# learningmatter-mit/surface-sampling

Hardware: AMD Instinct MI355X
Metric: MC energy-evaluations/sec (SrTiO3(001) ~250-atom slabs, 3-model PaiNN ensemble E+F incl. neighbor list) (higher is better)
Workload: dtype f32 via fp16x2-split MFMA (3 products), fp32 accumulate; neighbor decisions f64; 1 GPU; SrTiO3(001) PaiNN x3, 256 batched independent chains per GPU (BASELINE configs[3]), 248-272 atoms/chain; chains_per_gpu=256, atoms_per_gpu=66503, edges_per_gpu=2747786, slots_per_gpu=2836316, models=3, streams_per_gpu=2, parallelism=one GPU, no collective

## Files before the change

### surface-sampling_amd/csrc/api_painn.hip

```cpp
#include <cmath>

#include "vssr_internal.h"

namespace vssr {

static void transpose(const float *src, int rows, int cols, float *dst) {
    for (int r = 0; r < rows; ++r)
        for (int c = 0; c < cols; ++c) dst[(size_t)c * rows + r] = src[(size_t)r * cols + c];
}

static int upload_weights(vssr_handle *h, const vssr_painn_config *cfg) {
    const int M = cfg->n_models, L = cfg->num_conv, R = cfg->n_rbf, H = cfg->readout_hidden, NE = cfg->n_embed;
    const size_t per_layer = (size_t)F * F + F + (size_t)F3 * F + F3 + (size_t)F3 * R + F3 + 2 * (size_t)F * F +
                             (size_t)F * 2 * F + F + (size_t)F3 * F + F3;
    const size_t blob_len = (size_t)NE * F + L * per_layer + (size_t)H * F + H + H + 1;
    if (cfg->weights_len != blob_len)
        return set_err(h, VSSR_E_BADARG, "weights_len %llu does not match the layout (%zu floats)",
                       (unsigned long long)cfg->weights_len, blob_len);
    const size_t t_per_layer = (size_t)F * F + (size_t)F * F3 + 2 * (size_t)F * F + (size_t)2 * F * F + (size_t)F * F3;
    const size_t img_len = blob_len + L * t_per_layer + (size_t)F * H;
    std::vector<float> img(img_len * M);
    std::vector<ModelW> table(M);
    if (h->weights.ensure(img.size() * sizeof(float)))
        return set_err(h, VSSR_E_NOMEM, "weights: out of device memory");
// ... 83 lines not shown
        for (int m = 0; m < M; ++m) {
            const float *hb = img.data() + (size_t)m * img_len;
            size_t o = (size_t)NE * F;
            for (int l = 0; l < L; ++l) {
                const float *Wd = hb + o + (size_t)F * F + F + (size_t)F3 * F + F3;
                build_wd16(Wd, Wd + (size_t)F3 * 20, w16.data() + ((size_t)m * L + l) * per_layer16);
                o += per_layer;
            }
        }
        if (h->wd16.ensure(w16.size() * sizeof(unsigned))) return set_err(h, VSSR_E_NOMEM, "split filter weights");
        VSSR_HIP(h, hipMemcpy(h->wd16.p, w16.data(), w16.size() * sizeof(unsigned), hipMemcpyHostToDevice));
        for (int m = 0; m < M; ++m)
            for (int l = 0; l < L; ++l)
                table[m].layer[l].wd16 = h->wd16.as<uint4>() + ((size_t)m * L + l) * per_layer16 / 4;
    }
    {
        const size_t per_model = (size_t)NE * 2 * 24 * F;
        std::vector<float> A(per_model * M), At(per_model * M);
        for (int m = 0; m < M; ++m) {
            const float *hb = img.data() + (size_t)m * img_len;
            size_t o = (size_t)NE * F;
            const float *W1 = hb + o; o += (size_t)F * F;
            const float *b1 = hb + o; o += F;
            const float *W2 = hb + o; o += (size_t)F3 * F;
            const float *b2 = hb + o; o += F3;
            const float *Wd = hb + o; o += (size_t)F3 * R;
            const float *bd = hb + o;
            l0_build_tables(hb, W1, b1, W2, b2, Wd, bd, NE, A.data() + per_model * m, At.data() + per_model * m);
        }
        const size_t pk = l0_packed_dwords(NE);
        std::vector<unsigned> A16(pk * M), At16(pk * M);
        for (int m = 0; m < M; ++m) l0_pack_tables(A.data() + per_model * m, NE, A16.data() + pk * m, At16.data() + pk * m);
        if (h->d_l0A.ensure(A16.size() * sizeof(unsigned)) || h->d_l0At.ensure(At16.size() * sizeof(unsigned)))
            return set_err(h, VSSR_E_NOMEM, "layer-0 tables");
        VSSR_HIP(h, hipMemcpy(h->d_l0A.p, A16.data(), A16.size() * sizeof(unsigned), hipMemcpyHostToDevice));
        VSSR_HIP(h, hipMemcpy(h->d_l0At.p, At16.data(), At16.size() * sizeof(unsigned), hipMemcpyHostToDevice));
    }
    if (h->model_table.ensure(sizeof(ModelW) * M)) return set_err(h, VSSR_E_NOMEM, "model table");
    VSSR_HIP(h, hipMemcpy(h->model_table.p, table.data(), sizeof(ModelW) * M, hipMemcpyHostToDevice));
    return VSSR_OK;
}

}

using namespace vssr;

extern "C" {

int vssr_create(const vssr_painn_config *cfg, vssr_handle **out) {
    if (!cfg || !out) return set_err(nullptr, VSSR_E_BADARG, "null argument");
    *out = nullptr;
    if (cfg->struct_size != sizeof(vssr_painn_config))
        return set_err(nullptr, VSSR_E_BADARG, "vssr_painn_config size mismatch (%u vs %zu)", cfg->struct_size,
                       sizeof(vssr_painn_config));
    if (cfg->feat_dim < 16 || cfg->feat_dim > 256 || cfg->feat_dim % 16 != 0 || cfg->n_rbf < 1 || cfg->n_rbf > 32)
        return set_err(nullptr, VSSR_E_BADARG,
                       "feat_dim must be a multiple of 16 in 16..256 and n_rbf in 1..32 (got %d, %d)", cfg->feat_dim, cfg->n_rbf);
    if (cfg->n_models < 1 || cfg->n_models > MAX_MODELS || cfg->num_conv < 1 || cfg->num_conv > MAX_LAYERS ||
        cfg->readout_hidden < 1 || cfg->readout_hidden > F || cfg->n_embed < 1 || !cfg->weights ||
        !(cfg->cutoff > 0) || !(cfg->model_units_per_ev > 0))
        return set_err(nullptr, VSSR_E_BADARG, "bad PaiNN configuration");
    if (cfg->excl_vol && (cfg->excl_power < 1 || cfg->excl_power > 64 || !(cfg->excl_sigma > 0)))
        return set_err(nullptr, VSSR_E_BADARG, "excluded volume: power %d (1 .. 64) / sigma %g out of range", cfg->excl_power,
                       (double)cfg->excl_sigma);
    return create_handle(Kind::PAINN, cfg->device, out, [cfg](vssr_handle *h) {
        h->n_models = cfg->n_models; h->n_rbf = cfg->n_rbf; h->num_conv = cfg->num_conv; h->n_embed = cfg->n_embed;
        h->readout_hidden = cfg->readout_hidden; h->cutoff = cfg->cutoff; h->excl_vol = cfg->excl_vol;
        h->excl_power = cfg->excl_power; h->excl_sigma = cfg->excl_sigma; h->units_per_ev = cfg->model_units_per_ev;
        h->feat_dim = cfg->feat_dim;
        h->painn_general = !(cfg->feat_dim == F && cfg->n_rbf == 20);
        if (const char *e = getenv("VSSR_PAINN_PATH")) h->painn_general = h->painn_general || strcmp(e, "general") == 0;
        int rc = VSSR_OK;
        if (h->painn_general) {
            h->l0_enabled = 0;
            rc = painn_gen_upload(h, cfg);
        } else {
            rc = upload_weights(h, cfg);
            if (!rc) rc = node_mfma_init(h);
            if (!rc) rc = edge_mfma_init(h);
            if (!rc) rc = l0_mfma_init(h);
        }
        if (const char *e = getenv("VSSR_EDGE_IMPL")) h->edge_impl = (strcmp(e, "gather") == 0) ? 0 : 1;
        if (const char *e = getenv("VSSR_L0_FACTORISE")) h->l0_enabled = h->painn_general ? 0 : atoi(e);
        if (const char *e = getenv("VSSR_UPD_SAVE")) h->upd_save = atoi(e);
        if (const char *e = getenv("VSSR_DEBUG_KEEP")) h->debug_keep = atoi(e);
        if (const char *e = getenv("VSSR_EDGE_FS16_MAX")) h->fs16_max_atoms = atoi(e);
        if (const char *e = getenv("VSSR_EDGE_FS8_MAX")) h->fs8_max_atoms = atoi(e);
        if (const char *e = getenv("VSSR_EDGE_BWD_MPASS")) h->bwd_multi_pass = atoi(e);
        if (const char *e = getenv("VSSR_EDGE_SUB_CHUNK")) { const int c = atoi(e); if (c >= 8) { h->sub_chunk_fwd = c; h->sub_chunk_bwd = c; } }
        if (const char *e = getenv("VSSR_EDGE_FWD_2PASS")) { const int w = atoi(e); h->fwd_two_pass = (w == 8 || w == 16) ? w : w ? 16 : 0; }
        if (!rc && cfg->offset_per_z) {
            h->has_offset = true;
            h->offset_const = cfg->offset_const;
            if (h->offset_per_z.ensure(sizeof(double) * cfg->n_embed)) rc = set_err(h, VSSR_E_NOMEM, "offset table");
            else if (hipMemcpy(h->offset_per_z.p, cfg->offset_per_z, sizeof(double) * cfg->n_embed,
                               hipMemcpyHostToDevice) != hipSuccess)
                rc = set_err(h, VSSR_E_DEVICE, "offset table upload failed");
        }
        return rc;
    });
}

}
```

### surface-sampling_amd/csrc/painn.hip

```cpp
#include "vssr_internal.h"

namespace vssr {

constexpr int T = NODE_TILE;
constexpr int RB = 21;
constexpr int ECHUNK = 16;
constexpr float PI_F = 3.14159265358979323846f;

__device__ inline float sigmoidf_(float x) { return 1.f / (1.f + expf(-x)); }
__device__ inline float swishf_(float x) { return x * sigmoidf_(x); }
__device__ inline float dswishf_(float x) {
    float sg = sigmoidf_(x);
    return sg * fmaf(x, 1.f - sg, 1.f);
}

__global__ void __launch_bounds__(128) k_embed(int N, const int *__restrict__ Z, const ModelW *__restrict__ MW,
                                               float *__restrict__ s0, float *__restrict__ v0) {
    int i = blockIdx.x, m = blockIdx.y, f = threadIdx.x;
    const ModelW &W = MW[m];
    size_t a = (size_t)m * N + i;
    s0[a * F + f] = W.embed[(size_t)Z[i] * F + f];
    v0[(a * 3 + 0) * F + f] = 0.f;
    v0[(a * 3 + 1) * F + f] = 0.f;
    v0[(a * 3 + 2) * F + f] = 0.f;
// ... 504 lines not shown
    sv.n_atoms = (int)N;
    sv.n_models = (int)M;
    for (size_t l = 0; l <= L; ++l) { sv.s_in[l] = p; p += nS; sv.v_in[l] = p; p += nV; }
    for (size_t l = 0; l < L; ++l) {
        sv.phi[l] = p; p += nP;
        sv.s_msg[l] = p; p += nS;
        sv.v_msg[l] = p; p += nV;
    }
    sv.e_atom = p; p += M * N;
    sv.sbar = p; p += nS;
    sv.vbar = p; p += nV;
    sv.sbar_msg = p; p += nS;
    sv.vbar_msg = p; p += nV;
    sv.phibar = p; p += nP;
    if (h->upd_save && readout_mfma_supported(h->readout_hidden) &&
        h->d_upd_save.ensure(update_save_bytes((int)N, (int)M) * L))
        return set_err(h, VSSR_E_NOMEM, "forward intermediates of the update blocks: out of device memory");
    const size_t groups = (size_t)painn_gbar_groups(h);
    const bool compact = h->gbar_mode == 2 && groups > 1;
    if (h->d_gbar.ensure(sizeof(float4) * M * (compact ? 1 : groups) * (size_t)h->slot_cap) ||
        (compact && h->d_gpart.ensure(sizeof(float) * 3 * M * groups * (size_t)h->slot_cap + 256)))
        return set_err(h, VSSR_E_NOMEM, "edge-gradient buffer: out of device memory");
    sv.gbar = h->d_gbar.as<float4>();
    return painn_alloc_results(h);
}

int painn_alloc_results(vssr_handle *h) {
    const size_t N = h->n_atoms, M = h->n_models;
    if (h->d_energy.ensure(sizeof(float) * h->n_cfg) || h->d_energy_std.ensure(sizeof(float) * h->n_cfg) ||
        h->d_energy_models.ensure(sizeof(float) * h->n_cfg * M) || h->d_energy64.ensure(sizeof(double) * h->n_cfg * (2 + M)) ||
        h->d_forces.ensure(sizeof(float) * 3 * N) ||
        h->d_forces_std.ensure(sizeof(float) * 3 * N) || h->d_e_atoms.ensure(sizeof(float) * N))
        return set_err(h, VSSR_E_NOMEM, "result buffers: out of device memory");
    if (h->d_sat.bytes < sizeof(unsigned) * h->n_cfg || h->d_sat_out.bytes < sizeof(unsigned) * h->n_cfg) {
        if (h->d_sat.ensure(sizeof(unsigned) * h->n_cfg) || h->d_sat_out.ensure(sizeof(unsigned) * h->n_cfg))
            return set_err(h, VSSR_E_NOMEM, "saturation flags: out of device memory");
        VSSR_HIP(h, hipMemsetAsync(h->d_sat.p, 0, h->d_sat.bytes, h->stream));
        VSSR_HIP(h, hipMemsetAsync(h->d_sat_out.p, 0, h->d_sat_out.bytes, h->stream));
    }
    return VSSR_OK;
}

int painn_run(vssr_handle *h, uint32_t want) {
    if (h->painn_general) return painn_gen_run(h, want);
    const int N = h->n_atoms, M = h->n_models, L = h->num_conv, H = h->readout_hidden;
    hipStream_t st = h->stream;
    h->h_sat_valid = false;
    int rc = build_neighbors(h, (double)h->cutoff);
    if (rc) return rc;
    rc = painn_alloc_state(h);
    if (rc) return rc;
    StateView &sv = h->sv;
    sv.e_excl = h->d_excl.as<float>();
    GraphView G;
    G.n_atoms = N;
    G.n_cfg = h->n_cfg;
    G.atom_cfg = h->d_atom_cfg.as<int>();
    G.cfg_start = h->d_cfg_start.as<int>();
    G.row_start = h->d_row_start.as<int>();
    G.deg = h->d_deg.as<int>();
    G.edge = h->d_edge.as<float4>();
    G.rev = h->d_rev.as<int>();
    G.erec = h->d_erec.as<float4>();
    G.rho = h->d_rho.as<float>();
    G.dist2 = h->d_dist.as<float2>();
    G.rho16 = h->d_rho16.as<uint4>();
    G.drho16 = h->d_drho16.as<uint4>();
    G.zslot = h->d_zslot.as<unsigned char>();
    G.bundle = h->d_bundle.as<int4>();
    G.chain_class = h->d_chain_class.as<unsigned char>();
    G.act = ActiveView{h->active_mask, h->d_atom_cfg.as<int>(), h->d_sat.as<unsigned>()};
    const ActiveView &av = G.act;
    const ModelW *MW = h->model_table.as<ModelW>();
    const int *counters = h->d_counters.as<int>();
    const int *Z = h->d_Z.as<int>();
    dim3 blk(128);
    dim3 g_atom(N, M), g_tile((N + T - 1) / T, M);
    Profiler &P = h->prof;
    const bool l0_fact = h->l0_enabled && h->l0_nz > 0;
    const int n_groups = painn_gbar_groups(h);
    const int layer_sets = n_groups > 1 ? gbar_layer_sets(h) : 1;
    const bool compact = h->gbar_mode == 2 && n_groups > 1;
    const int fin_groups = compact ? 1 : n_groups;
    const int *cls_list[EDGE_MFMA_CLASSES];
    const int *bcls_list[EDGE_MFMA_BCLASSES];
    {
        int o = 0;
        for (int c = 0; c < EDGE_MFMA_CLASSES; o += h->n_class[c], ++c) cls_list[c] = h->d_class_list.as<int>() + o;
        for (int c = 0; c < EDGE_MFMA_BCLASSES; o += h->n_bclass[c], ++c) bcls_list[c] = h->d_class_list.as<int>() + o;
    }
    const int n_gather = h->n_class[EDGE_CLASS_GATHER];
    const bool keep = h->upd_save && (want & VSSR_WANT_FORCES) && readout_mfma_supported(H);
    auto save_of = [&](int l) -> void * { return keep ? (char *)h->d_upd_save.p + update_save_bytes(N, M) * (size_t)l : nullptr; };
    h->l0_used = l0_fact;

    if (!l0_fact) {
        P.begin(KC_EMBED, st);
        hipLaunchKernelGGL(k_embed, g_atom, blk, 0, st, N, Z, MW, sv.s_in[0], sv.v_in[0]);
        P.end(st);
    }
    for (int l = 0; l < L; ++l) {
        if (l == 0 && l0_fact) {
            P.begin(KC_L0_FWD, st);
            rc = l0_run_forward(h, G, sv.s_msg[0], sv.v_msg[0]);
            if (rc) return rc;
            P.end(st);
            P.begin(KC_UPDATE_FWD, st);
            launch_update_fwd_mfma(st, N, M, l, av, MW, sv.s_msg[l], sv.v_msg[l], sv.s_in[l + 1],
                                   (l + 1 < L || h->debug_keep) ? sv.v_in[l + 1] : nullptr, l + 1 < L ? sv.phi[l + 1] : nullptr, save_of(l));
            P.end(st);
            continue;
        }
        if (l == 0) {
            P.begin(KC_MSG_MLP, st);
            launch_msg_mlp_mfma(st, N, M, l, av, MW, sv.s_in[l], sv.phi[l]);
            P.end(st);
        }
        P.begin(KC_EDGE_FWD, st);
        if (l == 0)
            hipLaunchKernelGGL(k_edge_fwd<true>, g_atom, blk, 0, st, N, l, MW, G, counters, h->cutoff, h->excl_vol,
                               h->excl_sigma, h->excl_power, sv.s_in[l], sv.v_in[l], sv.phi[l], sv.s_msg[l],
                               sv.v_msg[l], -1);
        else {
            for (int cls = 0; cls < EDGE_MFMA_CLASSES; ++cls)
                launch_edge_fwd_mfma(st, cls, N, cls_list[cls], h->n_class[cls], M, l, h->max_class_atoms[cls], MW, G, counters,
                                     (int)(h->slot_cap - 1), sv.s_in[l], sv.v_in[l], sv.phi[l], sv.s_msg[l], sv.v_msg[l],
                                     (cls == EDGE_CLASS_FS4 && h->fwd_two_pass) ? h->d_bundle_sub.as<int4>() : (const int4 *)nullptr,
                                     h->fwd_two_pass, h->sub_chunk_fwd ? h->sub_chunk_fwd : sub_chunk_max(h->fwd_two_pass));
            if (n_gather)
                hipLaunchKernelGGL(k_edge_fwd<false>, g_atom, blk, 0, st, N, l, MW, G, counters, h->cutoff, h->excl_vol,
                                   h->excl_sigma, h->excl_power, sv.s_in[l], sv.v_in[l], sv.phi[l], sv.s_msg[l],
                                   sv.v_msg[l], (int)EDGE_BCLASS_GATHER);
        }
        P.end(st);
        P.begin(KC_UPDATE_FWD, st);
        launch_update_fwd_mfma(st, N, M, l, av, MW, sv.s_msg[l], sv.v_msg[l], sv.s_in[l + 1],
                               (l + 1 < L || h->debug_keep) ? sv.v_in[l + 1] : nullptr, l + 1 < L ? sv.phi[l + 1] : nullptr, save_of(l));
        P.end(st);
    }
    const bool fused = readout_mfma_supported(H);
    const bool want_forces = (want & VSSR_WANT_FORCES) != 0;
    const float *e_excl = h->excl_vol ? sv.e_excl : (const float *)nullptr;
    if (!(fused && want_forces)) {
        P.begin(KC_READOUT, st);
        if (fused) launch_readout_mfma(st, N, M, av, MW, sv.s_in[L], e_excl, sv.e_atom);
        else
            hipLaunchKernelGGL(k_readout, g_tile, blk, 0, st, N, H, av, MW, sv.s_in[L], sv.e_excl, h->excl_vol, sv.e_atom,
                               sv.sbar);
        P.end(st);
    }

    if (want_forces) {
        float *sb_buf[2] = {sv.sbar_msg, sv.sbar};
        for (int l = L - 1; l >= 0; --l) {
            float *sbar_msg_l = fused ? sb_buf[(L - 1 - l) & 1] : sv.sbar_msg;
            const float *sbar_msg_up = sb_buf[(L - l) & 1];
            P.begin(KC_UPDATE_BWD, st);
            if (!fused)
                launch_update_bwd_mfma(st, N, M, l, 0, (int)(l == L - 1), av, MW, sv.s_msg[l], sv.v_msg[l], sv.sbar, sv.vbar,
                                       nullptr, nullptr, nullptr, nullptr, sbar_msg_l, sv.vbar_msg, nullptr);
            else if (l == L - 1)
                launch_update_bwd_mfma(st, N, M, l, 1, 1, av, MW, sv.s_msg[l], sv.v_msg[l], nullptr, sv.vbar, sv.s_in[L], nullptr,
                                       e_excl, sv.e_atom, sbar_msg_l, sv.vbar_msg, save_of(l));
            else
                launch_update_bwd_mfma(st, N, M, l, 2, 0, av, MW, sv.s_msg[l], sv.v_msg[l], sbar_msg_up, sv.vbar, sv.s_in[l + 1],
                                       sv.phibar, nullptr, nullptr, sbar_msg_l, sv.vbar_msg, save_of(l));
            P.end(st);
            sv.sbar_msg_l0 = sbar_msg_l;
            P.begin((l == 0 && l0_fact) ? KC_L0_BWD : KC_EDGE_BWD, st);
            int accumulate = (l != L - 1);
            if (l == 0 && l0_fact) {
                rc = l0_run_reverse(h, G, (int)(L == 1), (int)compact, sbar_msg_l, sv.vbar_msg, sv.gbar, (long long)h->slot_cap,
                                    fin_groups);
                if (rc) return rc;
            } else if (l == 0)
                hipLaunchKernelGGL(k_edge_bwd<true>, g_atom, blk, 0, st, N, l, accumulate, MW, G, counters,
                                   h->cutoff, h->excl_vol, h->excl_sigma, h->excl_power, sv.v_in[l], sv.phi[l],
                                   sbar_msg_l, sv.vbar_msg, sv.phibar, sv.vbar, sv.gbar,
                                   (long long)h->slot_cap * fin_groups, -1, (int)compact);
            else {
                if ((l == L - 1 || layer_sets > 1) && !compact && h->n_cfg > n_gather)
                    return set_err(h, VSSR_E_STATE, "matrix-pipe reverse kernels need the compact partial-gradient records");
                for (int cls = 0; cls < EDGE_MFMA_BCLASSES; ++cls)
                    launch_edge_bwd_mfma(st, cls, N, bcls_list[cls], h->n_bclass[cls], M, l, (int)(l == L - 1 || layer_sets > 1),
                                         h->max_bclass_atoms[cls], MW, G, counters, (int)(h->slot_cap - 1), sv.v_in[l], sv.phi[l],
                                         sbar_msg_l, sv.vbar_msg, sv.phibar, sv.vbar,
                                         compact ? h->d_gpart.as<float>() : reinterpret_cast<float *>(sv.gbar), (long long)h->slot_cap,
                                         n_groups, layer_sets > 1 ? (L - 1 - l) * (n_groups / layer_sets) : 0, compact ? 3 : 4,
                                         cls == EDGE_BCLASS_FS16P ? h->d_bundle_subb.as<int4>() : (const int4 *)nullptr,
                                         h->sub_chunk_bwd ? h->sub_chunk_bwd : sub_chunk_max_bwd());
                if (n_gather)
                    hipLaunchKernelGGL(k_edge_bwd<false>, g_atom, blk, 0, st, N, l, accumulate, MW, G, counters,
                                       h->cutoff, h->excl_vol, h->excl_sigma, h->excl_power, sv.v_in[l], sv.phi[l],
                                       sbar_msg_l, sv.vbar_msg, sv.phibar, sv.vbar, sv.gbar,
                                       (long long)h->slot_cap * fin_groups, (int)EDGE_BCLASS_GATHER, 0);
            }
            P.end(st);
            if (l > 0 && !fused) {
                P.begin(KC_MSG_MLP_BWD, st);
                launch_msg_mlp_bwd_mfma(st, N, M, l, av, MW, sv.s_in[l], sv.phibar, sv.sbar_msg, sv.sbar);
                P.end(st);
            }
        }
    }
    P.begin(KC_FINALIZE, st);
    if (want & VSSR_WANT_FORCES) {
#ifdef ABL_LDS_FORCE
        if (compact) {
        } else if (false) {
#else
        if (compact) {
#endif
            const int uni = h->active_mask ? 0 : h->n_bclass[EDGE_BCLASS_FS16] + h->n_bclass[EDGE_BCLASS_FS16P] == h->n_cfg ? 8 : h->n_bclass[EDGE_BCLASS_FS8] == h->n_cfg ? 16
                            : h->n_bclass[EDGE_BCLASS_FS4] == h->n_cfg ? 32 : 0;
            const dim3 grid = uni ? dim3((unsigned)((h->slot_cap + 255) / 256), 1) : dim3(h->n_cfg, 12);
            hipLaunchKernelGGL(k_reduce_gpart, grid, dim3(256), 0, st, M, n_groups, layer_sets, G, counters, h->d_gpart.as<float>(),
                               sv.gbar, (long long)h->slot_cap, uni);
        } else if (n_groups > 1) {
            const int cls_only = h->n_bclass[EDGE_BCLASS_FS16] + h->n_bclass[EDGE_BCLASS_FS16P] == h->n_cfg ? EDGE_BCLASS_FS16
                                 : h->n_bclass[EDGE_BCLASS_FS8] == h->n_cfg ? EDGE_BCLASS_FS8
                                 : h->n_bclass[EDGE_BCLASS_FS4] == h->n_cfg ? EDGE_BCLASS_FS4 : -1;
            if (cls_only >= 0 && !h->active_mask && (layer_sets == 1 || n_gather == 0))
                hipLaunchKernelGGL(k_reduce_gbar_groups_uniform, dim3((unsigned)((h->slot_cap + 255) / 256)), dim3(256), 0, st, M,
                                   n_groups, counters, sv.gbar, (long long)h->slot_cap);
            else
                hipLaunchKernelGGL(k_reduce_gbar_groups, dim3(h->n_cfg, 12), dim3(256), 0, st, M, n_groups, layer_sets, G, counters, sv.gbar,
                                   (long long)h->slot_cap);
        }
        hipLaunchKernelGGL(k_finalize_forces, dim3((N + 3) / 4), dim3(256), 0, st, N, M, G, counters, sv.gbar,
                           (long long)h->slot_cap * fin_groups, h->units_per_ev, h->d_forces.as<float>(),
                           h->d_forces_std.as<float>());
    }
    hipLaunchKernelGGL(k_finalize_energy, dim3(h->n_cfg), dim3(256), 0, st, N, M, h->active_mask, G.cfg_start, Z, sv.e_atom,
                       h->units_per_ev, h->has_offset ? h->offset_per_z.as<double>() : (const double *)nullptr,
                       h->offset_const, h->d_energy.as<float>(), h->d_energy_std.as<float>(),
                       h->d_energy_models.as<float>(), h->d_energy64.as<double>(), h->d_e_atoms.as<float>(),
                       h->d_sat.as<unsigned>(), h->d_sat_out.as<unsigned>());
    P.end(st);
    VSSR_HIP(h, hipGetLastError());
    return VSSR_OK;
}

void painn_finalize(vssr_handle *h, const GraphView &G, uint32_t want, long long gbar_model_stride) {
    const int N = h->n_atoms, M = h->n_models;
    hipStream_t st = h->stream;
    if (want & VSSR_WANT_FORCES)
        hipLaunchKernelGGL(k_finalize_forces, dim3((N + 3) / 4), dim3(256), 0, st, N, M, G, h->d_counters.as<int>(), h->sv.gbar,
                           gbar_model_stride, h->units_per_ev, h->d_forces.as<float>(), h->d_forces_std.as<float>());
    hipLaunchKernelGGL(k_finalize_energy, dim3(h->n_cfg), dim3(256), 0, st, N, M, h->active_mask, G.cfg_start, h->d_Z.as<int>(),
                       h->sv.e_atom, h->units_per_ev, h->has_offset ? h->offset_per_z.as<double>() : (const double *)nullptr,
                       h->offset_const, h->d_energy.as<float>(), h->d_energy_std.as<float>(), h->d_energy_models.as<float>(),
                       h->d_energy64.as<double>(), h->d_e_atoms.as<float>(), h->d_sat.as<unsigned>(), h->d_sat_out.as<unsigned>());
}

int painn_stress(vssr_handle *h) {
    if (h->d_stress.ensure(sizeof(double) * 12 * (size_t)h->n_cfg)) return set_err(h, VSSR_E_DEVICE, "out of device memory (stress)");
    GraphView G{};
    G.n_atoms = h->n_atoms;
    G.n_cfg = h->n_cfg;
    G.cfg_start = h->d_cfg_start.as<int>();
    G.row_start = h->d_row_start.as<int>();
    G.edge = h->d_edge.as<float4>();
    const int fin_groups = h->gbar_mode == 2 ? 1 : painn_gbar_groups(h);
    double *out = h->d_stress.as<double>();
    hipLaunchKernelGGL(k_stress, dim3(h->n_cfg), dim3(256), 0, h->stream, h->n_models, G, h->d_counters.as<int>(), h->sv.gbar,
                       (long long)h->slot_cap * fin_groups, h->d_cell.as<double>(), h->units_per_ev, out, out + 6 * (size_t)h->n_cfg);
    VSSR_HIP(h, hipGetLastError());
    return VSSR_OK;
}

}
```

### surface-sampling_amd/csrc/painn_l0.hip

```cpp
#include "mfma16.h"

namespace vssr {

constexpr int KP = 24;
constexpr int TBLK = 4 * KP;

template <int NZ>
__global__ void __launch_bounds__(96)
k_l0_accum(GraphView G, const int *__restrict__ counters, float *__restrict__ T) {
    constexpr int nz = NZ;
    if (counters[2] || !G.act.atom(blockIdx.x)) return;
    const int i = blockIdx.x, comp = threadIdx.x / KP, kap = threadIdx.x % KP;
    float acc[NZ];
#pragma unroll
    for (int z = 0; z < NZ; ++z) acc[z] = 0.f;
    auto erec_c = [&](int idx) -> float4 {
#if defined(__HIP_DEVICE_COMPILE__)
        typedef const f32x4 __attribute__((address_space(4))) *cp;
        const f32x4 v = reinterpret_cast<cp>(reinterpret_cast<uintptr_t>(G.erec))[idx];
        return make_float4(v.x, v.y, v.z, v.w);
#else
        return G.erec[idx];
#endif
    };
// ... 169 lines not shown
                    const int a_ = a0 + 16 * tt + 4 * g + i;
                    if (a_ < N) Q[((((size_t)m * N + a_) * nz + q) * 4 + comp) * KP + kap] = acc[t][i];
                }
            }
        }
    }
}

__global__ void __launch_bounds__(256)
k_l0_bwd(int N, int M, int nz, int first_write, int fresh_mfma, int excl_vol, float rc, GraphView G, const int *__restrict__ counters,
         const float *__restrict__ Q, float4 *__restrict__ gbar, long long gbar_group_stride, int n_groups) {
    extern __shared__ __attribute__((aligned(16))) float qs_all[];
    const int lane = threadIdx.x & 63, wave = threadIdx.x >> 6, sl = lane >> 2, kq = lane & 3;
    const int n = blockIdx.x * (blockDim.x >> 6) + wave;
    if (n >= N || counters[2] || !G.act.atom(n)) return;
    const int per_model = nz * TBLK;
    const bool fw = first_write || (fresh_mfma && G.chain_class[G.atom_cfg[n]] != EDGE_BCLASS_GATHER);
    float *qs = qs_all + (size_t)wave * M * per_model;
    for (int m = 0; m < M; ++m) {
        const float4 *src = reinterpret_cast<const float4 *>(Q + ((size_t)m * N + n) * per_model);
        for (int i = lane; i < per_model / 4; i += 64) reinterpret_cast<float4 *>(qs + m * per_model)[i] = src[i];
    }
    __builtin_amdgcn_fence(__ATOMIC_RELEASE, "wavefront");
    __builtin_amdgcn_wave_barrier();
    __builtin_amdgcn_fence(__ATOMIC_ACQUIRE, "wavefront");
    const int e0 = G.row_start[n], e1 = G.row_start[n + 1];
    for (int eb = e0; eb < e1; eb += 16) {
        const int e = min(eb + sl, e1 - 1);
        const bool live = eb + sl < e1;
        const float4 ed = G.edge[e];
        const float2 dd = G.dist2[e];
        const int zi = G.zslot[e];
        const int re = G.rev[e];
        float rho[6], drho[6], inv;
        bool valid;
        radial_quarter(ed, kq, rc, rho, drho, inv, valid);
        const float4 er = make_float4(ed.x * inv, ed.y * inv, ed.z * inv, 0.f);
        const bool real = live && zi < nz && re >= 0 && valid;
        const int zq = zi < nz ? zi : 0;
        for (int m = 0; m < M; ++m) {
            const float *q = qs + m * per_model + zq * TBLK + kq * 6;
            float qv[4][6];
#pragma unroll
            for (int cq = 0; cq < 4; ++cq)
#pragma unroll
                for (int k = 0; k < 3; ++k) {
                    const float2 t2 = reinterpret_cast<const float2 *>(q + cq * KP)[k];
                    qv[cq][2 * k] = t2.x; qv[cq][2 * k + 1] = t2.y;
                }
            float d0 = 0.f, dx = 0.f, dy = 0.f, dz = 0.f, bx = 0.f, by = 0.f, bz = 0.f;
#pragma unroll
            for (int k = 0; k < 6; ++k) {
                const float q0 = qv[0][k], qx = qv[1][k], qy = qv[2][k], qz = qv[3][k];
                d0 = fmaf(drho[k], q0, d0);
                dx = fmaf(drho[k], qx, dx); dy = fmaf(drho[k], qy, dy); dz = fmaf(drho[k], qz, dz);
                bx = fmaf(rho[k], qx, bx); by = fmaf(rho[k], qy, by); bz = fmaf(rho[k], qz, bz);
            }
            auto qsum = [](float x) {
                x += __builtin_bit_cast(float, __builtin_amdgcn_update_dpp(0, __builtin_bit_cast(int, x), 0xB1, 0xF, 0xF, true));
                x += __builtin_bit_cast(float, __builtin_amdgcn_update_dpp(0, __builtin_bit_cast(int, x), 0x4E, 0xF, 0xF, true));
                return x;
            };
            d0 = qsum(d0); dx = qsum(dx); dy = qsum(dy); dz = qsum(dz); bx = qsum(bx); by = qsum(by); bz = qsum(bz);
            if (real && kq == 0) {
                const float ux = -er.x, uy = -er.y, uz = -er.z;
                float db = d0 - (dx * ux + dy * uy + dz * uz);
                if (excl_vol) db += dd.y;
                const float invd = inv;
                const float dotu = fmaf(bz, uz, fmaf(by, uy, bx * ux));
                float g0 = fmaf(-db, ux, (bx - dotu * ux) * invd);
                float g1 = fmaf(-db, uy, (by - dotu * uy) * invd);
                float g2 = fmaf(-db, uz, (bz - dotu * uz) * invd);
                float4 *gb = gbar + (size_t)m * n_groups * gbar_group_stride;
                if (!fw) {
                    const float4 old = gb[re];
                    g0 += old.x; g1 += old.y; g2 += old.z;
                }
                gb[re] = make_float4(g0, g1, g2, 0.f);
            }
        }
    }
}

void l0_build_tables(const float *blob_embed, const float *W1, const float *b1, const float *W2, const float *b2,
                     const float *Wd, const float *bd, int n_embed, float *A ,
                     float *At ) {
    std::vector<float> h(F), phi(F3);
    for (int z = 0; z < n_embed; ++z) {
        const float *s = blob_embed + (size_t)z * F;
        for (int o = 0; o < F; ++o) {
            float acc = b1[o];
            for (int k = 0; k < F; ++k) acc = fmaf(W1[(size_t)o * F + k], s[k], acc);
            h[o] = acc / (1.f + expf(-acc));
        }
        for (int o = 0; o < F3; ++o) {
            float acc = b2[o];
            for (int k = 0; k < F; ++k) acc = fmaf(W2[(size_t)o * F + k], h[k], acc);
            phi[o] = acc;
        }
        for (int sec = 0; sec < 2; ++sec)
            for (int kap = 0; kap < KP; ++kap) {
                const int kq = kap / 6, ks = kap % 6;
                const int k = ks < 5 ? kq + 4 * ks : (kq == 0 ? 20 : 99);
                for (int f = 0; f < F; ++f) {
                    const int row = (sec + 1) * F + f;
                    const float w = k < 20 ? Wd[(size_t)row * 20 + k] : (k == 20 ? bd[row] : 0.f);
                    const float val = phi[row] * w;
                    A[(((size_t)z * 2 + sec) * KP + kap) * F + f] = val;
                    At[(((size_t)z * 2 + sec) * F + f) * KP + kap] = val;
                }
            }
    }
}

void l0_pack_tables(const float *A , int n_embed, unsigned *A16, unsigned *At16) {
    std::vector<float> fk((size_t)F * 32), kf((size_t)32 * F);
    for (int z = 0; z < n_embed; ++z)
        for (int sec = 0; sec < 2; ++sec) {
            std::fill(fk.begin(), fk.end(), 0.f);
            std::fill(kf.begin(), kf.end(), 0.f);
            for (int kap = 0; kap < KP; ++kap)
                for (int f = 0; f < F; ++f) {
                    const float v = A[(((size_t)z * 2 + sec) * KP + kap) * F + f];
                    fk[(size_t)f * 32 + kap] = v;
                    kf[(size_t)kap * F + f] = v;
                }
            const size_t o = ((size_t)z * 2 + sec) * L0_TILE_U4 * 4;
            pack_mfma_tiles16(fk.data(), F, 32, A16 + o);
            pack_mfma_tiles16(kf.data(), 32, F, At16 + o);
        }
}
size_t l0_packed_dwords(int n_embed) { return (size_t)n_embed * 2 * L0_TILE_U4 * 4; }

int l0_mfma_init(vssr_handle *h) {
    VSSR_HIP(h, hipFuncSetAttribute((const void *)k_l0_fwd16, hipFuncAttributeMaxDynamicSharedMemorySize, 160 * 1024));
    VSSR_HIP(h, hipFuncSetAttribute((const void *)k_l0_q16, hipFuncAttributeMaxDynamicSharedMemorySize, 160 * 1024));
    return VSSR_OK;
}

int l0_run_forward(vssr_handle *h, const GraphView &G, float *s_msg, float *v_msg) {
    const int N = h->n_atoms, M = h->n_models, nz = h->l0_nz;
    hipStream_t st = h->stream;
    if (h->d_l0T.ensure(sizeof(float) * (size_t)N * nz * TBLK) ||
        h->d_l0Q.ensure(sizeof(float) * (size_t)M * N * nz * TBLK))
        return set_err(h, VSSR_E_NOMEM, "layer-0 factorisation buffers: out of device memory");
    if (!h->l0T_by_geom) {
        const int *cnt = h->d_counters.as<int>();
        float *T = h->d_l0T.as<float>();
        switch (nz) {
            case 1: hipLaunchKernelGGL(k_l0_accum<1>, dim3(N), dim3(96), 0, st, G, cnt, T); break;
            case 2: hipLaunchKernelGGL(k_l0_accum<2>, dim3(N), dim3(96), 0, st, G, cnt, T); break;
            case 3: hipLaunchKernelGGL(k_l0_accum<3>, dim3(N), dim3(96), 0, st, G, cnt, T); break;
            case 4: hipLaunchKernelGGL(k_l0_accum<4>, dim3(N), dim3(96), 0, st, G, cnt, T); break;
            case 5: hipLaunchKernelGGL(k_l0_accum<5>, dim3(N), dim3(96), 0, st, G, cnt, T); break;
            case 6: hipLaunchKernelGGL(k_l0_accum<6>, dim3(N), dim3(96), 0, st, G, cnt, T); break;
            case 7: hipLaunchKernelGGL(k_l0_accum<7>, dim3(N), dim3(96), 0, st, G, cnt, T); break;
            default: hipLaunchKernelGGL(k_l0_accum<L0_MAX_SPECIES>, dim3(N), dim3(96), 0, st, G, cnt, T); break;
        }
    }
    const size_t lds_fwd = sizeof(_Float16) * (plane_halves(TA, 32 * nz) + plane_halves(3 * TA, 32 * nz));
    hipLaunchKernelGGL(k_l0_fwd16, dim3((N + TA - 1) / TA), dim3(NTHREADS), lds_fwd, st, N, M, nz, G.act, h->d_counters.as<int>(),
                       h->d_Z.as<int>(), h->d_zlist.as<int>(), h->model_table.as<ModelW>(), h->d_l0A.as<uint4>(), h->n_embed,
                       h->d_l0T.as<float>(), s_msg, v_msg);
    return VSSR_OK;
}

int l0_run_reverse(vssr_handle *h, const GraphView &G, int first_write, int fresh_mfma, const float *sbar_msg, const float *vbar_msg,
                   float4 *gbar, long long gbar_stride, int n_groups) {
    const int N = h->n_atoms, M = h->n_models, nz = h->l0_nz;
    hipStream_t st = h->stream;
    const size_t lds_q = sizeof(_Float16) * (plane_halves(TA, F) + plane_halves(3 * TA, F));
    hipLaunchKernelGGL(k_l0_q16, dim3((N + TA - 1) / TA, M), dim3(NTHREADS), lds_q, st, N, nz, G.act, h->d_counters.as<int>(),
                       h->d_zlist.as<int>(), h->d_l0At.as<uint4>(), h->n_embed, sbar_msg, vbar_msg, h->d_l0Q.as<float>());
    if (sizeof(float) * 4 * M * nz * TBLK > 48 * 1024)
        VSSR_HIP(h, hipFuncSetAttribute((const void *)k_l0_bwd, hipFuncAttributeMaxDynamicSharedMemorySize, 160 * 1024));
    hipLaunchKernelGGL(k_l0_bwd, dim3((N + 3) / 4), dim3(256), sizeof(float) * 4 * M * nz * TBLK, st, N, M, nz, first_write, fresh_mfma,
                       h->excl_vol, h->cutoff, G, h->d_counters.as<int>(), h->d_l0Q.as<float>(), gbar, gbar_stride, n_groups);
    return VSSR_OK;
}

}
```

### surface-sampling_amd/csrc/vssr_internal.h

```cpp
#pragma once

#include <hip/hip_runtime.h>

#include <cstdint>
#include <cstdio>
#include <cstdlib>
#include <cstring>
#include <memory>
#include <string>
#include <utility>
#include <vector>

#include "../../include/vssr_eval.h"

namespace vssr {

constexpr int F = 128;
constexpr int F3 = 3 * F;
constexpr int MAX_LAYERS = 4;
constexpr int MAX_MODELS = 8;
constexpr int RB_MAX = 24;
constexpr int NODE_TILE = 8;
constexpr int L0_MAX_SPECIES = 8;

// ... 229 lines not shown
struct Cluster {
    int n_components = 0, whiten = 1, d_clu = 3, d_pad = 3;
    bool pca_done = false;
    int64_t n_pts = 0;
    DevBuf mean, denom, part_sum, part_cov, cov, evec, eval, comp, comp_t, ev, ratio, jac, xr;
    DevBuf pts;
    DevBuf cen[2], siz[2], cid[2];
    DevBuf nn, flag, blk, rec, counters;
};

enum class Kind : int {
    NONE = 0,
    PAINN = 1,
    TERSOFF = 2,
    EAM = 3,
    SW = 4,
    GMM = 5,
    GMM_FIT = 6,
    CLUSTER = 7,
    PAIR = 8,
    COUNT
};
constexpr unsigned kind_bit(Kind k) { return 1u << (int)k; }
constexpr unsigned KINDS_EVAL = kind_bit(Kind::PAINN) | kind_bit(Kind::TERSOFF) | kind_bit(Kind::EAM) | kind_bit(Kind::SW) |
                                kind_bit(Kind::PAIR);

}

struct vssr_handle {
    vssr::Kind kind = vssr::Kind::NONE;
    vssr_eam_grid eam_grid = {0, 0, 0.0, 0.0, 0.0};
    int eam_nel = 0, eam_fs = 0;
    int device = 0;
    vssr::OwnedStream stream;
    std::string err;
    vssr::Profiler prof;

    int edge_impl = 1;
    int max_cfg_atoms = 0;
    vssr::DevBuf d_chain_class, d_class_list;
    int n_class[5] = {0, 0, 0, 0, 0}, max_class_atoms[5] = {0, 0, 0, 0, 0};
    int n_bclass[5] = {0, 0, 0, 0, 0}, max_bclass_atoms[5] = {0, 0, 0, 0, 0};
    int fs16_max_atoms = -1, fs8_max_atoms = -1, fs4_max_atoms = -1;
    int max_images = 0;

    int n_models = 0, n_rbf = 20, num_conv = 3, n_embed = 100, readout_hidden = 64;
    int feat_dim = vssr::F;
    bool painn_general = false;
    float cutoff = 5.f;
    int excl_vol = 1, excl_power = 12;
    float excl_sigma = 1.5f;
    double units_per_ev = 1.0;
    bool has_offset = false;
    double offset_const = 0.0;

    vssr::DevBuf weights;
    vssr::DevBuf wd16;
    vssr::DevBuf node16;
    vssr::DevBuf model_table;
    vssr::DevBuf offset_per_z;

    int n_types = 0;
    double pot_cutoff = 0;
    bool ew_on = false;
    double ew_g = 0, ew_kcut = 0, ew_q[8] = {0, 0, 0, 0, 0, 0, 0, 0};
    int ew_stride = 0;
    vssr::DevBuf d_ew_S;
    vssr::DevBuf pot_params;

    bool batch_valid = false, ran = false;
    int n_cfg = 0, n_atoms = 0;
    std::vector<int> h_n_atoms, h_cfg_start;
    vssr::DevBuf d_pos, d_wpos, d_wrap, d_Z, d_atom_cfg, d_cfg_start, d_cell, d_invcell, d_nimg, d_pbc;
    vssr::DevBuf d_deg, d_row_start, d_edge, d_edge_S, d_rev, d_counters, d_tile_sums;
    vssr::DevBuf d_erec, d_rho, d_dist, d_rho16, d_drho16, d_zslot, d_bundle, d_excl;
    vssr::DevBuf d_bundle_sub;
    int bwd_multi_pass = 1;
    int fwd_mpass_fs8 = 1;
    int sub_chunk_fwd = 0, sub_chunk_bwd = 0;
    vssr::DevBuf d_bundle_subb;
    int fwd_two_pass = 16;
    vssr::DevBuf d_hits;
    int l0_enabled = 1, l0_nz = 0;
    bool l0_used = false;
    vssr::DevBuf d_l0A, d_l0At;
    vssr::DevBuf d_zmap, d_zlist;
    vssr::DevBuf d_l0T, d_l0Q;
    vssr::DevBuf d_opt_state, d_opt_vec, d_bfgs_q, d_bfgs_b, d_fixed, d_relax_steps, d_relax_conv, d_active;
    const unsigned char *active_mask = nullptr;
    int relax_regrows = 0;
    long long relax_lockstep = 0;
    int relax_compactions = 0;
    vssr::DevBuf d_cmp;
    vssr::DevBuf d_cm;
    long long relax_chain_evals = 0;
    int traj_interval = 0, traj_records = 0, traj_B = 0, traj_N = 0;
    vssr::DevBuf d_traj_pos, d_traj_f, d_traj_e, d_traj_n;
    bool graph_partial = false;
    bool l0T_by_geom = false;
    int64_t zero_entry_cap = -1;
    const void *zero_entry_tab[2] = {nullptr, nullptr};
    int cap_per_atom = 64;
    int cm_cap_per_atom = 0;
    int cg_driver = 0;
    int cg_last_driver = 0;
    bool cap_tight = false;
    uint32_t last_want = 0;
    int64_t slot_cap = 0;
    vssr::PinnedInts h_counters;

    vssr::DevBuf d_state;
    vssr::StateView sv;
    vssr::DevBuf d_gbar;
    vssr::DevBuf d_upd_save;
    int gbar_mode = 2;
    vssr::DevBuf d_gpart;
    int debug_keep = 0;
    int upd_save = 0;
    vssr::DevBuf d_energy, d_energy_std, d_energy_models, d_forces, d_forces_std, d_e_atoms;
    vssr::DevBuf d_energy64;
    vssr::DevBuf d_pot_e, d_pot_ea, d_pot_f;
    vssr::DevBuf d_sat, d_sat_out;
    std::vector<unsigned> h_sat;
    bool h_sat_valid = false;
    vssr::DevBuf d_stress;

    int gmm_K = 0, gmm_D = 0, gmm_Dp = 0;
    double gmm_log2pi = 0.0;
    vssr::DevBuf d_gmm_P;
    vssr::DevBuf d_gmm_c;
    vssr::DevBuf d_gmm_kc;
    vssr::DevBuf d_gmm_mask;
    vssr::DevBuf d_gmm_x, d_gmm_lp, d_gmm_nll, d_gmm_sys, d_gmm_start;
    std::unique_ptr<vssr::GmmFit> fit;
    std::unique_ptr<vssr::Cluster> clu;
};

namespace vssr {

int set_err(vssr_handle *h, int code, const char *fmt, ...);
#define VSSR_HIP(h, expr)                                                                    \
    do {                                                                                     \
        hipError_t _e = (expr);                                                              \
        if (_e != hipSuccess)                                                                \
            return vssr::set_err(h, VSSR_E_DEVICE, "%s failed: %s (%s:%d)", #expr,          \
                                 hipGetErrorString(_e), __FILE__, __LINE__);                 \
    } while (0)

int check_kind(vssr_handle *h, unsigned served, const char *func);
int device_in_range(vssr_handle *h, int device);
int open_device(vssr_handle *h, int device);
void publish_create_error(const vssr_handle *h);
template <class Init>
int create_handle(Kind kind, int device, vssr_handle **out, Init init, bool range_check = true) {
    vssr_handle *h = new vssr_handle();
    h->kind = kind;
    int rc = range_check ? device_in_range(h, device) : VSSR_OK;
    if (!rc) rc = open_device(h, device);
    if (!rc) rc = init(h);
    if (rc) {
        publish_create_error(h);
        vssr_destroy(h);
        return rc;
    }
    *out = h;
    return VSSR_OK;
// ... 3 lines not shown
int grow_slot_cap(vssr_handle *h);

int build_neighbors(vssr_handle *h, double cutoff);
int painn_alloc_state(vssr_handle *h);
int painn_run(vssr_handle *h, uint32_t want);
int painn_stress(vssr_handle *h);
int painn_alloc_results(vssr_handle *h);
void painn_finalize(vssr_handle *h, const GraphView &G, uint32_t want, long long gbar_model_stride);
int painn_gen_upload(vssr_handle *h, const vssr_painn_config *cfg);
int painn_gen_run(vssr_handle *h, uint32_t want);
int tersoff_run(vssr_handle *h, uint32_t want);
int eam_run(vssr_handle *h, uint32_t want);
int sw_run(vssr_handle *h, uint32_t want);
int pair_run(vssr_handle *h, uint32_t want);
int gmm_upload(vssr_handle *g, const double *means, const double *prec_chol, const double *weights);
int gmm_score_f64(vssr_handle *g, hipStream_t st, int64_t n, const double *x_dev);
int gmm_score_f32(vssr_handle *g, hipStream_t st, int64_t n, const float *x_dev);
int gmm_mean_rows(vssr_handle *g, hipStream_t st, int B, const int *start, const float *emb);
int gmm_reduce(vssr_handle *g, hipStream_t st, int B, const int *start, int order);
int gmm_fit_check_config(const vssr_gmm_fit_config *cfg);
int gmm_fit_append_host(vssr_handle *h, int64_t n_rows, const double *x);
int gmm_fit_append_f32(vssr_handle *h, hipStream_t st, int64_t n_rows, const float *emb_dev);
int gmm_fit_append_f64p(vssr_handle *h, hipStream_t st, int64_t n_rows, const double *x_dev);
int gmm_fit_set_init(vssr_handle *h, const double *means, const double *weights, const double *precisions, const int32_t *labels);
int gmm_fit_run(vssr_handle *h, vssr_gmm_fit_result *res);
int gmm_fit_params(vssr_handle *h, double *weights, double *means, double *covariances, double *prec_chol);
int gmm_fit_copy_scorer(vssr_handle *h, vssr_handle *g);
int gmm_fit_centered_cov(vssr_handle *h, hipStream_t st, const double *X, int n, int D, int Dp, const double *mean, const double *denom,
                         DevBuf &part, double *cov);
int cluster_pca(vssr_handle *h, vssr_cluster_pca_result *res);
int cluster_pca_params(vssr_handle *h, double *mean, double *components, double *explained_variance, double *ratio);
int cluster_projected(vssr_handle *h, int64_t first, int64_t n_rows, double *xr);
int cluster_set_points(vssr_handle *h, int64_t n, const double *pts);
int cluster_linkage(vssr_handle *h, double *Z, int32_t *n_rounds);
int cluster_pad_dims(int d);
int tersoff_stress(vssr_handle *h);
int eam_stress(vssr_handle *h);
int sw_stress(vssr_handle *h);
struct PotView;
void ewald_run(vssr_handle *h, const PotView &V);
int ewald_stress(vssr_handle *h);
int pair_stress(vssr_handle *h);
struct Evaluator {
    bool f64;
    int (*run)(vssr_handle *h, uint32_t want);
    int (*stress)(vssr_handle *h);
    double (*cutoff)(const vssr_handle *h);
};
const Evaluator &evaluator(const vssr_handle *h);
inline bool is_analytic(const vssr_handle *h) { return evaluator(h).f64; }
void eam_build_spline(const double *f, int n, double delta, double *spl );
int relax_fire(vssr_handle *h, const vssr_fire_params &p, const uint8_t *fixed_host, uint32_t want);
int relax_bfgs(vssr_handle *h, const vssr_bfgs_params &p, const uint8_t *fixed_host, uint32_t want);
int relax_begin(vssr_handle *h, const uint8_t *fixed_host, int steps_ints_per_chain, const uint8_t *&fixed);
int relax_regrow(vssr_handle *h, int cap, long long &it, int window);
int relax_cg(vssr_handle *h, const vssr_cg_params *cp, const uint8_t *fixed_host, uint32_t want);
int relax_bfgsls(vssr_handle *h, const vssr_bfgsls_params *bp, const uint8_t *fixed_host, uint32_t want);
bool chain_min_supported(const vssr_handle *h);
int chain_min_cg(vssr_handle *h, const vssr_cg_params *cp, const uint8_t *fixed_host, uint32_t want);
int node_mfma_init(vssr_handle *h);
void launch_msg_mlp_mfma(hipStream_t st, int N, int M, int l, const ActiveView &av, const ModelW *MW, const float *s_in,
                         float *phi);
void launch_msg_mlp_bwd_mfma(hipStream_t st, int N, int M, int l, const ActiveView &av, const ModelW *MW, const float *s_in,
                             const float *phibar, const float *sbar_msg, float *sbar_in);
void launch_update_fwd_mfma(hipStream_t st, int N, int M, int l, const ActiveView &av, const ModelW *MW, const float *s_msg,
                            const float *v_msg, float *s_out, float *v_out, float *phi_next, void *save);
size_t update_save_bytes(int N, int M);
bool readout_mfma_supported(int hidden);
void launch_readout_mfma(hipStream_t st, int N, int M, const ActiveView &av, const ModelW *MW, const float *s, const float *e_excl,
                         float *e_atom);
void launch_update_bwd_mfma(hipStream_t st, int N, int M, int l, int mode, int vbar_is_zero, const ActiveView &av, const ModelW *MW,
                            const float *s_msg, const float *v_msg, const float *sbar_src, const float *vbar,
                            const float *s_next, const float *phibar, const float *e_excl, float *e_atom,
                            float *sbar_msg, float *vbar_msg, const void *save);
void pack_mfma_tiles16(const float *Wsrc, int rows, int K, unsigned *dst );
void build_wd16(const float *Wd, const float *bd, unsigned *dst );
void l0_build_tables(const float *blob_embed, const float *W1, const float *b1, const float *W2, const float *b2,
                     const float *Wd, const float *bd, int n_embed, float *A, float *At);
void l0_pack_tables(const float *A, int n_embed, unsigned *A16, unsigned *At16);
size_t l0_packed_dwords(int n_embed);
int l0_mfma_init(vssr_handle *h);
int l0_run_forward(vssr_handle *h, const GraphView &G, float *s_msg, float *v_msg);
int l0_run_reverse(vssr_handle *h, const GraphView &G, int first_write, int fresh_mfma, const float *sbar_msg, const float *vbar_msg,
                   float4 *gbar, long long gbar_stride, int n_groups);
int edge_mfma_init(vssr_handle *h);
enum { EDGE_CLASS_FS16 = 0, EDGE_CLASS_FS16M = 1, EDGE_CLASS_FS8 = 2, EDGE_CLASS_FS4 = 3, EDGE_CLASS_GATHER = 4, EDGE_CLASSES = 5,
       EDGE_MFMA_CLASSES = 4 };
enum { EDGE_BCLASS_FS16 = 0, EDGE_BCLASS_FS8 = 1, EDGE_BCLASS_FS4 = 2, EDGE_BCLASS_FS16P = 3, EDGE_BCLASS_GATHER = 4, EDGE_BCLASSES = 5,
       EDGE_MFMA_BCLASSES = 4 };
__host__ __device__ constexpr int edge_bclass_slices(int c) { return (c == EDGE_BCLASS_FS16 || c == EDGE_BCLASS_FS16P) ? 8 : c == EDGE_BCLASS_FS8 ? 16 : c == EDGE_BCLASS_FS4 ? 32 : 1; }
int edge_bclass_of(int n_atoms);
int edge_class_of(int n_atoms);
constexpr int SUB_MAX_PASSES = 4;
__host__ __device__ constexpr int sub_chunk_max(int width) { return width == 16 ? 400 : 784; }
__host__ __device__ constexpr int sub_chunk_max_bwd() { return 550; }
__host__ __device__ constexpr int sub_passes(int n_atoms, int chunk_max) { return (n_atoms + chunk_max - 1) / chunk_max; }
__host__ __device__ constexpr int sub_chunk(int n_atoms, int chunk_max) { return (n_atoms + sub_passes(n_atoms, chunk_max) - 1) / sub_passes(n_atoms, chunk_max); }
int edge_class_groups(int cls);
void launch_edge_bwd_mfma(hipStream_t st, int cls, int N, const int *list, int n_list, int M, int l, int layer_first, int max_atoms,
                          const ModelW *MW, const GraphView &G, const int *counters, int zero_slot,
                          const float *v_in, const float *phi, const float *sbar_msg, const float *vbar_msg,
                          float *phibar, float *vbar_in, float *gbar, long long gbar_stride, int n_groups, int group_off, int rec,
                          const int4 *bundle_sub, int sub_chunk);
void launch_edge_fwd_mfma(hipStream_t st, int cls, int N, const int *list, int n_list, int M, int l, int max_atoms, const ModelW *MW,
                          const GraphView &G, const int *counters, int zero_slot, const float *s_in, const float *v_in,
                          const float *phi, float *s_msg, float *v_msg, const int4 *bundle_sub, int sub_width, int sub_chunk);

}
```

Measured before the change: 24800 evaluations/s.

## Fuse layer-0 reverse edge kernel with partial-gradient reduction, skipping finalize pass

Adds a k_l0_bwd_reduce kernel that computes the factorised layer-0 edge gradient and, in the same pass, sums the per-slice gradient partial records written by later layers, storing the final per-edge gbar directly. When enabled (on by default under compact gbar mode with L0 factorisation), the separate finalize reduction over the partial buffers is skipped. This removes one full read/write sweep over the edge-sized gbar arrays and a kernel launch. The cost is extra per-edge loads of up to layer_sets*slices records inside the L0 kernel, which can raise register pressure and memory latency there. Also adds an unused environment knob for the FS4 class threshold.

```diff
diff --git a/surface-sampling_amd/csrc/api_painn.hip b/surface-sampling_amd/csrc/api_painn.hip
--- a/surface-sampling_amd/csrc/api_painn.hip
+++ b/surface-sampling_amd/csrc/api_painn.hip
@@ -189,10 +189,12 @@
         }
         if (const char *e = getenv("VSSR_EDGE_IMPL")) h->edge_impl = (strcmp(e, "gather") == 0) ? 0 : 1;
         if (const char *e = getenv("VSSR_L0_FACTORISE")) h->l0_enabled = h->painn_general ? 0 : atoi(e);
+        if (const char *e = getenv("VSSR_L0_FUSED_REDUCE")) h->l0_fused_reduce = atoi(e);
         if (const char *e = getenv("VSSR_UPD_SAVE")) h->upd_save = atoi(e);
         if (const char *e = getenv("VSSR_DEBUG_KEEP")) h->debug_keep = atoi(e);
         if (const char *e = getenv("VSSR_EDGE_FS16_MAX")) h->fs16_max_atoms = atoi(e);
         if (const char *e = getenv("VSSR_EDGE_FS8_MAX")) h->fs8_max_atoms = atoi(e);
+        if (const char *e = getenv("VSSR_EDGE_FS4_MAX")) h->fs4_max_atoms = atoi(e);
         if (const char *e = getenv("VSSR_EDGE_BWD_MPASS")) h->bwd_multi_pass = atoi(e);
         if (const char *e = getenv("VSSR_EDGE_SUB_CHUNK")) { const int c = atoi(e); if (c >= 8) { h->sub_chunk_fwd = c; h->sub_chunk_bwd = c; } }
         if (const char *e = getenv("VSSR_EDGE_FWD_2PASS")) { const int w = atoi(e); h->fwd_two_pass = (w == 8 || w == 16) ? w : w ? 16 : 0; }
diff --git a/surface-sampling_amd/csrc/painn.hip b/surface-sampling_amd/csrc/painn.hip
--- a/surface-sampling_amd/csrc/painn.hip
+++ b/surface-sampling_amd/csrc/painn.hip
@@ -610,6 +610,7 @@
     const int layer_sets = n_groups > 1 ? gbar_layer_sets(h) : 1;
     const bool compact = h->gbar_mode == 2 && n_groups > 1;
     const int fin_groups = compact ? 1 : n_groups;
+    const bool fused_red = l0_fact && h->gbar_mode == 2 && h->l0_fused_reduce;
     const int *cls_list[EDGE_MFMA_CLASSES];
     const int *bcls_list[EDGE_MFMA_BCLASSES];
     {
@@ -699,7 +700,8 @@
             int accumulate = (l != L - 1);
             if (l == 0 && l0_fact) {
                 rc = l0_run_reverse(h, G, (int)(L == 1), (int)compact, sbar_msg_l, sv.vbar_msg, sv.gbar, (long long)h->slot_cap,
-                                    fin_groups);
+                                    fin_groups, (int)fused_red, compact ? h->d_gpart.as<float>() : (const float *)nullptr, n_groups,
+                                    compact ? layer_sets : 0);
                 if (rc) return rc;
             } else if (l == 0)
                 hipLaunchKernelGGL(k_edge_bwd<true>, g_atom, blk, 0, st, N, l, accumulate, MW, G, counters,
@@ -733,6 +735,8 @@
     }
     P.begin(KC_FINALIZE, st);
     if (want & VSSR_WANT_FORCES) {
+        if (fused_red) {
+        } else
 #ifdef ABL_LDS_FORCE
         if (compact) {
         } else if (false) {
diff --git a/surface-sampling_amd/csrc/painn_l0.hip b/surface-sampling_amd/csrc/painn_l0.hip
--- a/surface-sampling_amd/csrc/painn_l0.hip
+++ b/surface-sampling_amd/csrc/painn_l0.hip
@@ -275,6 +275,128 @@
     }
 }
 
+constexpr int L0_REC_CHUNK = 16;
+
+template <int SEL>
+__device__ __forceinline__ float quad_lane(float x) {
+    return __builtin_bit_cast(float, __builtin_amdgcn_update_dpp(0, __builtin_bit_cast(int, x), 0x55 * SEL, 0xF, 0xF, true));
+}
+
+__global__ void __launch_bounds__(256, 4)
+k_l0_bwd_reduce(int N, int M, int nz, int first_write, int excl_vol, float rc, GraphView G, const int *__restrict__ counters,
+                const float *__restrict__ Q, float4 *__restrict__ gbar, long long slot_cap, const float *__restrict__ P, int part_groups,
+                int layer_sets) {
+    extern __shared__ __attribute__((aligned(16))) float qs_all[];
+    const int lane = threadIdx.x & 63, wave = threadIdx.x >> 6, sl = lane >> 2, kq = lane & 3;
+    const int n = blockIdx.x * (blockDim.x >> 6) + wave;
+    if (n >= N || counters[2] || !G.act.atom(n)) return;
+    const int per_model = nz * TBLK;
+    const int slices = __builtin_amdgcn_readfirstlane(edge_bclass_slices(G.chain_class[G.atom_cfg[n]]));
+    const int n_rec = (slices > 1 && layer_sets > 0) ? layer_sets * slices : 0;
+    const int per_set = n_rec ? part_groups / layer_sets : 0, slice_sh = __builtin_ctz(slices);
+    const bool fw = first_write || n_rec > 0;
+    const size_t rec_stride = (size_t)slot_cap * 3;
+    const bool chunked = n_rec && per_set == slices && n_rec % L0_REC_CHUNK == 0;
+    float *qs = qs_all + (size_t)wave * M * per_model;
+    for (int m = 0; m < M; ++m) {
+        const float4 *src = reinterpret_cast<const float4 *>(Q + ((size_t)m * N + n) * per_model);
+        for (int i = lane; i < per_model / 4; i += 64) reinterpret_cast<float4 *>(qs + m * per_model)[i] = src[i];
+    }
+    __builtin_amdgcn_fence(__ATOMIC_RELEASE, "wavefront");
+    __builtin_amdgcn_wave_barrier();
+    __builtin_amdgcn_fence(__ATOMIC_ACQUIRE, "wavefront");
+    const int e0 = G.row_start[n], e1 = G.row_start[n + 1];
+    for (int eb = e0; eb < e1; eb += 16) {
+        const int e = min(eb + sl, e1 - 1);
+        const bool live = eb + sl < e1;
+        const float4 ed = G.edge[e];
+        const float2 dd = G.dist2[e];
+        const int zi = G.zslot[e];
+        const int re = G.rev[e];
+        const bool own = live && kq < 3;
+        auto load_recs = [&](int m, int c, float (&pv)[L0_REC_CHUNK]) {
+#pragma unroll
+            for (int u = 0; u < L0_REC_CHUNK; ++u) pv[u] = __builtin_nondeterministic_value(pv[u]);
+            if (own) {
+                const float *pm = P + ((size_t)(m * part_groups + c * L0_REC_CHUNK) * slot_cap + e) * 3 + kq;
+#pragma unroll
+                for (int u = 0; u < L0_REC_CHUNK; ++u, pm += rec_stride) pv[u] = *pm;
+            }
+        };
+        float rho[6], drho[6], inv;
+        bool valid;
+        radial_quarter(ed, kq, rc, rho, drho, inv, valid);
+        const float4 er = make_float4(ed.x * inv, ed.y * inv, ed.z * inv, 0.f);
+        const bool real = live && zi < nz && re >= 0 && valid;
+        const int zq = zi < nz ? zi : 0;
+        auto model = [&](int m, const float (&pv0)[L0_REC_CHUNK]) {
+            const float *q = qs + m * per_model + zq * TBLK + kq * 6;
+            float qv[4][6];
+#pragma unroll
+            for (int cq = 0; cq < 4; ++cq)
+#pragma unroll
+                for (int k = 0; k < 3; ++k) {
+                    const float2 t2 = reinterpret_cast<const float2 *>(q + cq * KP)[k];
+                    qv[cq][2 * k] = t2.x; qv[cq][2 * k + 1] = t2.y;
+                }
+            float d0 = 0.f, dx = 0.f, dy = 0.f, dz = 0.f, bx = 0.f, by = 0.f, bz = 0.f;
+#pragma unroll
+            for (int k = 0; k < 6; ++k) {
+                const float q0 = qv[0][k], qx = qv[1][k], qy = qv[2][k], qz = qv[3][k];
+                d0 = fmaf(drho[k], q0, d0);
+                dx = fmaf(drho[k], qx, dx); dy = fmaf(drho[k], qy, dy); dz = fmaf(drho[k], qz, dz);
+                bx = fmaf(rho[k], qx, bx); by = fmaf(rho[k], qy, by); bz = fmaf(rho[k], qz, bz);
+            }
+            auto qsum = [](float x) {
+                x += __builtin_bit_cast(float, __builtin_amdgcn_update_dpp(0, __builtin_bit_cast(int, x), 0xB1, 0xF, 0xF, true));
+                x += __builtin_bit_cast(float, __builtin_amdgcn_update_dpp(0, __builtin_bit_cast(int, x), 0x4E, 0xF, 0xF, true));
+                return x;
+            };
+            d0 = qsum(d0); dx = qsum(dx); dy = qsum(dy); dz = qsum(dz); bx = qsum(bx); by = qsum(by); bz = qsum(bz);
+            const float ux = -er.x, uy = -er.y, uz = -er.z;
+            float db = d0 - (dx * ux + dy * uy + dz * uz);
+            if (excl_vol) db += dd.y;
+            const float invd = inv;
+            const float dotu = fmaf(bz, uz, fmaf(by, uy, bx * ux));
+            const float g0 = fmaf(-db, ux, (bx - dotu * ux) * invd);
+            const float g1 = fmaf(-db, uy, (by - dotu * uy) * invd);
+            const float g2 = fmaf(-db, uz, (bz - dotu * uz) * invd);
+            const float g1_0 = quad_lane<0>(g1), g2_0 = quad_lane<0>(g2);
+            const float l0 = -(kq == 0 ? g0 : kq == 1 ? g1_0 : g2_0);
+            float4 *gb = gbar + (size_t)m * slot_cap;
+            float acc = real ? l0 : 0.f;
+            if (!fw) {
+                float old = 0.f;
+                if (own) old = reinterpret_cast<const float *>(gb + e)[kq];
+                acc = real ? l0 + old : old;
+            }
+            if (chunked) {
+#pragma unroll
+                for (int u = 0; u < L0_REC_CHUNK; ++u) acc += pv0[u];
+                for (int c = 1; c * L0_REC_CHUNK < n_rec; ++c) {
+                    float pv[L0_REC_CHUNK];
+                    load_recs(m, c, pv);
+#pragma unroll
+                    for (int u = 0; u < L0_REC_CHUNK; ++u) acc += pv[u];
+                }
+            } else if (n_rec) {
+                float rec = 0.f;
+                for (int j = 0; j < n_rec; ++j) {
+                    if (own) rec = P[((size_t)(m * part_groups + (j >> slice_sh) * per_set + (j & (slices - 1))) * slot_cap + e) * 3 + kq];
+                    acc += rec;
+                }
+            }
+            const float ay = quad_lane<1>(acc), az = quad_lane<2>(acc);
+            if (live && kq == 0 && (n_rec || real)) gb[e] = make_float4(acc, ay, az, 0.f);
+        };
+        for (int m = 0; m < M; ++m) {
+            float pv0[L0_REC_CHUNK];
+            if (chunked) load_recs(m, 0, pv0);
+            model(m, pv0);
+        }
+    }
+}
+
 void l0_build_tables(const float *blob_embed, const float *W1, const float *b1, const float *W2, const float *b2,
                      const float *Wd, const float *bd, int n_embed, float *A ,
                      float *At ) {
@@ -359,15 +481,23 @@
 }
 
 int l0_run_reverse(vssr_handle *h, const GraphView &G, int first_write, int fresh_mfma, const float *sbar_msg, const float *vbar_msg,
-                   float4 *gbar, long long gbar_stride, int n_groups) {
+                   float4 *gbar, long long gbar_stride, int n_groups, int fused, const float *gpart, int part_groups, int layer_sets) {
     const int N = h->n_atoms, M = h->n_models, nz = h->l0_nz;
     hipStream_t st = h->stream;
     const size_t lds_q = sizeof(_Float16) * (plane_halves(TA, F) + plane_halves(3 * TA, F));
     hipLaunchKernelGGL(k_l0_q16, dim3((N + TA - 1) / TA, M), dim3(NTHREADS), lds_q, st, N, nz, G.act, h->d_counters.as<int>(),
                        h->d_zlist.as<int>(), h->d_l0At.as<uint4>(), h->n_embed, sbar_msg, vbar_msg, h->d_l0Q.as<float>());
-    if (sizeof(float) * 4 * M * nz * TBLK > 48 * 1024)
+    const size_t lds = sizeof(float) * 4 * M * nz * TBLK;
+    if (fused) {
+        if (lds > 48 * 1024)
+            VSSR_HIP(h, hipFuncSetAttribute((const void *)k_l0_bwd_reduce, hipFuncAttributeMaxDynamicSharedMemorySize, 160 * 1024));
+        hipLaunchKernelGGL(k_l0_bwd_reduce, dim3((N + 3) / 4), dim3(256), lds, st, N, M, nz, first_write, h->excl_vol, h->cutoff, G,
+                           h->d_counters.as<int>(), h->d_l0Q.as<float>(), gbar, gbar_stride, gpart, part_groups, gpart ? layer_sets : 0);
+        return VSSR_OK;
+    }
+    if (lds > 48 * 1024)
         VSSR_HIP(h, hipFuncSetAttribute((const void *)k_l0_bwd, hipFuncAttributeMaxDynamicSharedMemorySize, 160 * 1024));
-    hipLaunchKernelGGL(k_l0_bwd, dim3((N + 3) / 4), dim3(256), sizeof(float) * 4 * M * nz * TBLK, st, N, M, nz, first_write, fresh_mfma,
+    hipLaunchKernelGGL(k_l0_bwd, dim3((N + 3) / 4), dim3(256), lds, st, N, M, nz, first_write, fresh_mfma,
                        h->excl_vol, h->cutoff, G, h->d_counters.as<int>(), h->d_l0Q.as<float>(), gbar, gbar_stride, n_groups);
     return VSSR_OK;
 }
diff --git a/surface-sampling_amd/csrc/vssr_internal.h b/surface-sampling_amd/csrc/vssr_internal.h
--- a/surface-sampling_amd/csrc/vssr_internal.h
+++ b/surface-sampling_amd/csrc/vssr_internal.h
@@ -335,6 +335,7 @@
     int fwd_two_pass = 16;
     vssr::DevBuf d_hits;
     int l0_enabled = 1, l0_nz = 0;
+    int l0_fused_reduce = 1;
     bool l0_used = false;
     vssr::DevBuf d_l0A, d_l0At;
     vssr::DevBuf d_zmap, d_zlist;
@@ -504,7 +505,7 @@
 int l0_mfma_init(vssr_handle *h);
 int l0_run_forward(vssr_handle *h, const GraphView &G, float *s_msg, float *v_msg);
 int l0_run_reverse(vssr_handle *h, const GraphView &G, int first_write, int fresh_mfma, const float *sbar_msg, const float *vbar_msg,
-                   float4 *gbar, long long gbar_stride, int n_groups);
+                   float4 *gbar, long long gbar_stride, int n_groups, int fused, const float *gpart, int part_groups, int layer_sets);
 int edge_mfma_init(vssr_handle *h);
 enum { EDGE_CLASS_FS16 = 0, EDGE_CLASS_FS16M = 1, EDGE_CLASS_FS8 = 2, EDGE_CLASS_FS4 = 3, EDGE_CLASS_GATHER = 4, EDGE_CLASSES = 5,
        EDGE_MFMA_CLASSES = 4 };
```

Result: no change. 25030 evaluations/s (median of 6 runs) (+0.9%).
